# omarezz46/BayesDLL

Measured on AMD Instinct MI355X. Metric: SG-HMC leapfrog steps/sec & HBM GB/s on ViT-L/32 params, 1/2/4/8 MI355X, higher is better.
Workload: dtype f32

## Files before the change

### bayesdll_amd/csrc/bdl_api.hip

```cpp
#include <algorithm>
#include "bdl_chain_common.hpp"
#include "bdl_claim_ring.hpp"
#include "bdl_measure.h"

#include <mutex>
#include <vector>

namespace bdl {
namespace {

thread_local std::string g_last_error;

int g_blocks_per_cu = 2;
int g_unroll = 1;
int g_grid_stride = 1;

int device_cu_count() {
  static int cached[64] = {0};
  int dev = 0;
  if (hipGetDevice(&dev) != hipSuccess || dev < 0 || dev >= 64) return 256;
  if (cached[dev] == 0) {
    int cus = 0;
    if (hipDeviceGetAttribute(&cus, hipDeviceAttributeMultiprocessorCount, dev) != hipSuccess ||
        cus <= 0)
// ... 479 lines not shown
  if (!s) return fail(BDL_ERR_NULL, "bdl_sgmcmc_step: null args");
  if (s->n < 0) return fail(BDL_ERR_ARG, "bdl_sgmcmc_step: n < 0");
  if (s->method < BDL_CSGHMC || s->method > BDL_SGLD_GRAD)
    return fail(BDL_ERR_ARG, "bdl_sgmcmc_step: unknown method");
  if (s->noise_mode < BDL_NOISE_NONE || s->noise_mode > BDL_NOISE_PHILOX)
    return fail(BDL_ERR_ARG, "bdl_sgmcmc_step: unknown noise mode");
  if (s->collect < BDL_COLLECT_NONE || s->collect > BDL_COLLECT_MEAN)
    return fail(BDL_ERR_ARG, "bdl_sgmcmc_step: unknown collect mode");
  if (s->n == 0) return BDL_OK;
  const bool grad_only = s->method == BDL_SGHMC_GRAD || s->method == BDL_SGLD_GRAD;
  const bool needs_mom = s->method == BDL_CSGHMC || s->method == BDL_SGHMC ||
                         s->method == BDL_SGHMC_GRAD ||
                         (s->method == BDL_SGLD && (s->flags & BDL_FLAG_MOMENTUM));
  const bool needs_prior = s->method != BDL_CSGHMC;
  if (!s->theta) return fail(BDL_ERR_NULL, "bdl_sgmcmc_step: theta is required");
  if (const int rc = check_runs_and_grad(s, "bdl_sgmcmc_step")) return rc;
  if (needs_mom && !s->mom) return fail(BDL_ERR_NULL, "bdl_sgmcmc_step: mom is required");
  if (needs_prior && !s->prior_mean)
    return fail(BDL_ERR_NULL, "bdl_sgmcmc_step: prior_mean is required for sghmc/sgld");
  if (s->noise_mode == BDL_NOISE_BUFFER && !s->noise)
    return fail(BDL_ERR_NULL, "bdl_sgmcmc_step: noise buffer is required");
  if (s->collect != BDL_COLLECT_NONE && !s->mom1)
    return fail(BDL_ERR_NULL, "bdl_sgmcmc_step: mom1 is required to collect");
  if (grad_only && s->collect != BDL_COLLECT_NONE)
    return fail(BDL_ERR_ARG, "bdl_sgmcmc_step: grad-only methods cannot collect");
  const void* ptrs[] = {s->theta, s->mom, s->prior_mean, s->noise, s->mom1, s->mom2};
  for (const void* p : ptrs)
    if (misaligned(p, 15)) return fail(BDL_ERR_ALIGN, "bdl_sgmcmc_step: vector not 16-B aligned");

  const int unroll = g_unroll;
  StepKernel k = bare ? (s->method == BDL_CSGHMC ? pick_step_csghmc_bare(s->collect, unroll)
                                                 : nullptr)
                      : pick_step(s->method, s->noise_mode, s->collect, unroll);
  if (!k) return fail(BDL_ERR_ARG, "bdl_sgmcmc_step: unsupported method/noise/collect combination");

  const int64_t ngroups = (s->n + 3) / 4;
  const int64_t per_iter = (int64_t)kBlock * unroll;
  const int64_t cap = (int64_t)device_cu_count() * g_blocks_per_cu;
  int64_t iters = (ngroups + per_iter - 1) / per_iter;
  int64_t grid = capped_grid(iters, cap);
  int64_t iters_per_block = (iters + grid - 1) / grid;
  grid = (iters + iters_per_block - 1) / iters_per_block;

  KArgs a;
  a.theta = s->theta;
  a.grad = s->grad;
  a.mom = s->mom;
  a.prior_mean = s->prior_mean;
  a.noise = s->noise;
  a.mom1 = s->mom1;
  a.mom2 = s->mom2;
  a.runs = s->runs;
  a.gbase = s->grad_base;
  a.nruns = s->nruns;
  a.flags = s->flags;
  a.n = s->n;
  const int order = drift ? drift->order : g_grid_stride;
  a.groups_per_block = order ? 0 : iters_per_block * per_iter;
  a.lr0 = s->lr[0];
  a.lr1 = s->lr[1];
  a.ns0 = s->noise_scale[0];
  a.ns1 = s->noise_scale[1];
  a.one_minus_alpha = s->one_minus_alpha;
  a.prior_sig = s->prior_sig;
  a.sigma2 = s->sigma2;
  a.n_data = s->n_data;
  a.mu = s->mu;
  a.ca = s->collect_a;
  a.cb = s->collect_b;
  a.seed = s->seed;
  a.chain = s->chain;
  a.step = s->step;
  a.clip = clip;
  a.nonfinite = s->nonfinite;
  a.goff = s->philox_offset;
  a.cgroups = (uint32_t)s->chain_groups;
  a.inv_s2 = recip_or(s->inv_sigma2, s->sigma2);
  a.inv_nd = recip_or(s->inv_n_data, s->n_data);
  a.inv_ca = recip_or(s->inv_collect_a, s->collect_a);
  a.inv_cb = recip_or(s->inv_collect_b, s->collect_b);

  int slot = -1;
  uint32_t* pair = nullptr;
  if (order == 2 && s->method == BDL_CSGHMC &&
      run_lds_bytes(s) + 16 <= (size_t)kMaxRuns * sizeof(bdl_run))
    pair = claim_pair(stream, &slot);
  g_last_order = pair ? 2 : (order ? 1 : 0);
  g_last_slot = slot;
  const int32_t citers = (int32_t)(BDL_CLAIM_GROUPS / per_iter);
  if (pair) grid = capped_grid((iters + citers - 1) / citers, cap);
  if (drift) {
    if (order == 2 && !pair)
      return fail(BDL_ERR_ARG, "bdl_sweep_drift: no counter pair for the dynamic order here");
    if (drift->record_bytes < grid * (int64_t)(BDL_DRIFT_WORDS * sizeof(uint64_t)))
      return fail(BDL_ERR_ARG, "bdl_sweep_drift: records too small for the launch's workgroups");
    *drift->grid = (int32_t)grid;
    hipLaunchKernelGGL(pick_drift(unroll, pair != nullptr), dim3((unsigned)grid), dim3(kBlock),
                       run_lds_bytes(s), stream, a, pair, citers, drift->records);
    return launched("bdl_sweep_drift");
  }
  if (pair) {
    hipLaunchKernelGGL(pick_step_csghmc_dyn(s->noise_mode, s->collect, unroll, bare),
                       dim3((unsigned)grid), dim3(kBlock), run_lds_bytes(s), stream, a, pair, citers);
    return launched("bdl_sgmcmc_step");
  }

  if (g_redirect_exec) {
    hipGraphNodeType nt = hipGraphNodeTypeEmpty;
    hipKernelNodeParams cur{};
    if (hipGraphNodeGetType(g_redirect_node, &nt) != hipSuccess || nt != hipGraphNodeTypeKernel ||
        hipGraphKernelNodeGetParams(g_redirect_node, &cur) != hipSuccess ||
        cur.func != (void*)k) {
      (void)hipGetLastError();
      return fail(BDL_ERR_ARG, "bdl_sgmcmc_step: the redirect node is not this step's kernel");
    }
    void* kp[] = {&a};
    hipKernelNodeParams p{};
    p.func = (void*)k;
    p.gridDim = dim3((unsigned)grid);
    p.blockDim = dim3(kBlock);
    p.sharedMemBytes = (unsigned)run_lds_bytes(s);
    p.kernelParams = kp;
    const hipError_t err = hipGraphExecKernelNodeSetParams(g_redirect_exec, g_redirect_node, &p);
    if (err != hipSuccess) {
      (void)hipGetLastError();
      g_last_error = std::string("bdl_sgmcmc_step: graph node update failed: ") +
                     hipGetErrorString(err);
      return BDL_ERR_LAUNCH;
    }
    return BDL_OK;
  }
  hipLaunchKernelGGL(k, dim3((unsigned)grid), dim3(kBlock), run_lds_bytes(s), stream, a);
  if (const int rc = launched("bdl_sgmcmc_step")) return rc;
  hipStreamCaptureStatus cs = hipStreamCaptureStatusNone;
  if (stream && hipStreamIsCapturing(stream, &cs) == hipSuccess &&
      cs == hipStreamCaptureStatusActive) {
    std::lock_guard<std::mutex> lk(g_captured_mu);
    if (std::find(g_captured_funcs.begin(), g_captured_funcs.end(), (const void*)k) ==
        g_captured_funcs.end())
      g_captured_funcs.push_back((const void*)k);
  }
  (void)hipGetLastError();
  return BDL_OK;
}


constexpr int kMixMaxR = 8, kMixMaxW = 6;
struct MixArgs {
  const float* r[kMixMaxR];
  float* w[kMixMaxW];
  int64_t n;
};

template <int NR, int U>
__device__ __forceinline__ void mix_load(const MixArgs& a, int64_t gb, f4v (&x)[U][NR]) {
#pragma unroll
  for (int u = 0; u < U; ++u) {
    const int64_t e = (gb + (int64_t)u * kBlock + threadIdx.x) * 4;
#pragma unroll
    for (int r = 0; r < NR; ++r) x[u][r] = vload(a.r[r] + e);
  }
}

template <int NR, int NW, int U, bool PACED>
__device__ __forceinline__ void mix_store(const MixArgs& a, int64_t gb, f4v (&x)[U][NR]) {
#pragma unroll
  for (int u = 0; u < U; ++u) {
    const int64_t gi = gb + (int64_t)u * kBlock + threadIdx.x;
    const int64_t e = gi * 4;
    f4v acc = x[u][0];
#pragma unroll
    for (int r = 1; r < NR; ++r) acc = acc + x[u][r] * 0.0f;
    if constexpr (PACED) acc = acc + philox_normal4((uint64_t)gi, 0x5eedull, 0, 1) * 0.0f;
#pragma unroll
    for (int w = 0; w < NW; ++w) vstore(a.w[w] + e, acc);
  }
}

template <int NR, int NW, int U, int S>
__global__ __launch_bounds__(kBlock) void bdl_mix_kernel(const MixArgs a) {
  constexpr int64_t kIter = (int64_t)kBlock * U;
  const int64_t ngroups = (a.n + 3) >> 2, nfull = a.n >> 2;
  const int64_t stride = (int64_t)gridDim.x * kIter;
  int64_t gb = (int64_t)blockIdx.x * kIter;
  if constexpr (S == BDL_MIX_PIPELINED) {
    f4v x[U][NR], y[U][NR];
// ... 525 lines not shown
```

### bayesdll_amd/csrc/bdl_kernels.hpp

```cpp
#pragma once
#include <hip/hip_runtime.h>

#include <stdint.h>
#include <stdio.h>
#include <string.h>

#include <algorithm>
#include <string>

#include "bdl_sgmcmc.h"
#include "bdl_order.h"

namespace bdl {

constexpr int kBlock = 256;

__device__ __forceinline__ uint4 philox4x32_10(uint4 c, uint32_t k0, uint32_t k1) {
#ifdef BDL_PHILOX_KEYS_PER_CALL
  asm volatile("" : "+s"(k0), "+s"(k1));
#endif
#if defined(BDL_PHILOX_ROUND_KEYS_PER_CALL) && !defined(BDL_PHILOX_KEYS_PER_CALL)
  asm volatile("" : "+s"(k0), "+s"(k1));
#endif
#pragma unroll
// ... 555 lines not shown
  f4v th[UNROLL], g[UNROLL], v[UNROLL], t0[UNROLL], ep[UNROLL], m1[UNROLL], m2[UNROLL];
  uint32_t at[UNROLL];
  float* gq[UNROLL];
  const f4v z = {0.f, 0.f, 0.f, 0.f};
  int rr = r0;
#pragma unroll
  for (int u = 0; u < UNROLL; ++u) {
    const int64_t e = (gb + (int64_t)u * kBlock + threadIdx.x) * 4;
    while (run_end(rr) <= e) ++rr;
    at[u] = run_attr(rr);
    gq[u] = run_grad(a, rr);
    v[u] = t0[u] = ep[u] = m1[u] = m2[u] = z;
    th[u] = vload(a.theta + e);
    g[u] = vload(gq[u] + e);
    if (T::kMom || (METHOD == BDL_SGLD && c.sgd_mom_read)) v[u] = vload(a.mom + e);
    if (T::kReadPrior) t0[u] = vload(a.prior_mean + e);
    if (NOISE == BDL_NOISE_BUFFER) ep[u] = vload(a.noise + e);
    if (T::kReadMoments) {
      m1[u] = vload(a.mom1 + e);
      if (c.has_m2) m2[u] = vload(a.mom2 + e);
    }
  }
#pragma unroll
  for (int u = 0; u < UNROLL; ++u) {
    const int64_t gi = gb + (int64_t)u * kBlock + threadIdx.x;
    const int64_t e = gi * 4;
    if constexpr (NOISE == BDL_NOISE_PHILOX) ep[u] = step_noise4(a, gi);
#pragma unroll
    for (int j = 0; j < 4; ++j) {
      float xt = th[u][j], xg = g[u][j], xv = v[u][j], x1 = m1[u][j], x2 = m2[u][j];
      update_elem<METHOD, NOISE, COLLECT, RECIP>(a, c, at[u], xt, xg, xv, t0[u][j], ep[u][j], x1,
                                                 x2);
      th[u][j] = xt;
      g[u][j] = xg;
      v[u][j] = xv;
      m1[u][j] = x1;
      m2[u][j] = x2;
    }
    if constexpr (T::kWriteTheta) {
      bad |= nonfinite4(th[u]);
      vstore(a.theta + e, th[u]);
    }
    if constexpr (T::kWriteGrad) {
      bad |= nonfinite4(g[u]);
      vstore(gq[u] + e, g[u]);
    }
    if (T::kMom || (METHOD == BDL_SGLD && c.sgd_mom)) vstore(a.mom + e, v[u]);
    if constexpr (T::kCollect) {
      vstore(a.mom1 + e, m1[u]);
      if (c.has_m2) vstore(a.mom2 + e, m2[u]);
    }
  }
}

constexpr int kVarGradReady = 1, kVarClip = 2, kVarRuntime = -1;

template <int COLLECT, int UNROLL>
constexpr bool csg_collect_per_run() {
  return UNROLL == 1 &&
         (COLLECT == BDL_COLLECT_WELFORD_INIT || COLLECT == BDL_COLLECT_MEAN_INIT);
}

template <int METHOD, int COLLECT, int VAR, class A>
__device__ __forceinline__ StepConst make_step_const(const A& a) {
  StepConst c;
  c.sgd_mom = (METHOD == BDL_SGLD) && (a.flags & BDL_FLAG_MOMENTUM);
  c.sgd_mom_read = c.sgd_mom && !(a.flags & BDL_FLAG_FIRST_STEP);
  c.has_m2 = (COLLECT != BDL_COLLECT_NONE) && (a.mom2 != nullptr);
  if constexpr (VAR == kVarRuntime) {
    c.grad_ready = (METHOD == BDL_SGLD || METHOD == BDL_SGHMC) && (a.flags & BDL_FLAG_GRAD_READY);
    c.clip = (METHOD == BDL_SGLD) && a.clip != nullptr;
  } else {
    c.grad_ready = (VAR & kVarGradReady) != 0;
    c.clip = (VAR & kVarClip) != 0;
  }
  c.clip_coef = c.clip ? a.clip[1] : 1.0f;
  c.inv_s2 = a.inv_s2;
  c.inv_nd = a.inv_nd;
  c.inv_ca = a.inv_ca;
  c.inv_cb = a.inv_cb;
  return c;
}

template <int METHOD, int NOISE, int COLLECT, bool RECIP, int UNROLL, int VAR>
__device__ __forceinline__ void step_body(const KArgs& a) {
  const StepConst c = make_step_const<METHOD, COLLECT, VAR>(a);

  const int64_t ngroups = (a.n + 3) >> 2;
  const int64_t nfull = a.n >> 2;
  constexpr int64_t kIter = (int64_t)kBlock * UNROLL;
  int64_t g0, g1, gstep;
  if (a.groups_per_block > 0) {
    g0 = (int64_t)blockIdx.x * a.groups_per_block;
    g1 = min(g0 + a.groups_per_block, ngroups);
    gstep = kIter;
  } else {
    g0 = (int64_t)blockIdx.x * kIter;
    g1 = ngroups;
    gstep = (int64_t)gridDim.x * kIter;
  }

  stage_runs(a);
  if (g0 >= g1) return;

  int r = find_run_lds(a.nruns, g0 * 4);
  uint32_t bad = 0;
  if constexpr (fresh_step_args<METHOD, NOISE, COLLECT, UNROLL>()) {
  for (int64_t gb = g0; gb < g1; gb += gstep) {
    ckargs& fa = fresh_kargs();
    const StepConst fc = make_step_const<METHOD, COLLECT, VAR>(fa);
    while (r < a.nruns - 1 && run_end(r) <= gb * 4) ++r;
    const int64_t gend = min(gb + kIter, g1);
    const uint32_t attr = run_attr(r);
    const bool full = gend == gb + kIter && gend <= nfull;
    if (full && run_end(r) >= gend * 4 && !(attr & kNoFastPath))
      chunk_fast_dispatch<METHOD, NOISE, COLLECT, RECIP, UNROLL>(fa, fc, gb, attr, run_grad(fa, r),
                                                                  bad);
    else if (full && multi_run_ok(a.nruns, r, gend * 4))
      chunk_multi<METHOD, NOISE, COLLECT, RECIP, UNROLL>(fa, fc, gb, r, bad);
    else
      chunk_slow<METHOD, NOISE, COLLECT, RECIP, UNROLL>(fa, fc, gb, gend, r, bad);
  }
  } else if constexpr (!is_csghmc_sweep<METHOD>() ||
                       (COLLECT != BDL_COLLECT_NONE && !csg_collect_per_run<COLLECT, UNROLL>())) {
  for (int64_t gb = g0; gb < g1; gb += gstep) {
    while (r < a.nruns - 1 && run_end(r) <= gb * 4) ++r;
    const int64_t gend = min(gb + kIter, g1);
    const uint32_t attr = run_attr(r);
    const bool full = gend == gb + kIter && gend <= nfull;
    if (full && run_end(r) >= gend * 4 && !(attr & kNoFastPath))
      chunk_fast_dispatch<METHOD, NOISE, COLLECT, RECIP, UNROLL>(a, c, gb, attr, run_grad(a, r),
                                                                  bad);
    else if (full && multi_run_ok(a.nruns, r, gend * 4))
      chunk_multi<METHOD, NOISE, COLLECT, RECIP, UNROLL>(a, c, gb, r, bad);
    else
      chunk_slow<METHOD, NOISE, COLLECT, RECIP, UNROLL>(a, c, gb, gend, r, bad);
  }
  } else {
  for (int64_t gb = g0; gb < g1;) {
    while (r < a.nruns - 1 && run_end(r) <= gb * 4) ++r;
    const uint32_t attr = run_attr(r);
    const int64_t lim = min(min(run_end(r) >> 2, nfull), g1);
    if (!(attr & kNoFastPath) && gb + kIter <= lim) {
      const bool head = (attr & BDL_ATTR_HEAD) != 0;
      gb = fast_run<METHOD, NOISE, COLLECT, RECIP, UNROLL, false, false>(
          a, c, gb, lim, gstep, head ? a.lr1 : a.lr0, head ? a.ns1 : a.ns0, run_grad(a, r), bad);
      continue;
    }
    const int64_t gend = min(gb + kIter, g1);
    if (gend == gb + kIter && gend <= nfull && multi_run_ok(a.nruns, r, gend * 4))
      chunk_multi<METHOD, NOISE, COLLECT, RECIP, UNROLL>(a, c, gb, r, bad);
    else
      chunk_slow<METHOD, NOISE, COLLECT, RECIP, UNROLL>(a, c, gb, gend, r, bad);
    gb += gstep;
  }
  }
  report_nonfinite(a, bad);
}

template <int METHOD, int NOISE, int COLLECT, bool RECIP, int UNROLL>
__device__ __forceinline__ void step_variant(const KArgs& a) {
  if constexpr (COLLECT != BDL_COLLECT_NONE || !(METHOD == BDL_SGLD || METHOD == BDL_SGHMC)) {
    step_body<METHOD, NOISE, COLLECT, RECIP, UNROLL, kVarRuntime>(a);
  } else {
    if (a.flags & BDL_FLAG_GRAD_READY)
      step_body<METHOD, NOISE, COLLECT, RECIP, UNROLL, kVarGradReady>(a);
    else if (METHOD == BDL_SGLD && a.clip != nullptr)
      step_body<METHOD, NOISE, COLLECT, RECIP, UNROLL, kVarClip>(a);
    else
      step_body<METHOD, NOISE, COLLECT, RECIP, UNROLL, 0>(a);
  }
}

template <int METHOD, int NOISE, int COLLECT, int UNROLL>
__global__ __launch_bounds__(kBlock) void bdl_step_kernel(const KArgs a) {
  if (a.flags & BDL_FLAG_RECIP_DIV)
    step_variant<METHOD, NOISE, COLLECT, true, UNROLL>(a);
  else
    step_variant<METHOD, NOISE, COLLECT, false, UNROLL>(a);
}

struct NoProbe {
  __device__ __forceinline__ void begin() {}
  __device__ __forceinline__ void tick(int64_t) {}
  __device__ __forceinline__ void end() {}
};

struct DriftProbe {
  uint64_t* __restrict__ rec;
  uint32_t it;
  __device__ __forceinline__ void begin() {
    if (threadIdx.x == 0) rec[0] = wall_clock64();
  }
  __device__ __forceinline__ void tick(int64_t iter) {
    if (it % BDL_DRIFT_EVERY == 0) {
      const uint32_t s = it / BDL_DRIFT_EVERY;
      if (s < BDL_DRIFT_SAMPLES && threadIdx.x == 0) {
        rec[4 + 2 * s] = wall_clock64();
        rec[5 + 2 * s] = (uint64_t)iter;
      }
    }
    ++it;
  }
  __device__ __forceinline__ void end() {
    __threadfence();
    __syncthreads();
    if (threadIdx.x == 0) {
      rec[1] = wall_clock64();
      rec[2] = min((it + BDL_DRIFT_EVERY - 1) / BDL_DRIFT_EVERY, (uint32_t)BDL_DRIFT_SAMPLES);
      rec[3] = it;
    }
  }
};

template <int METHOD, int NOISE, int COLLECT, bool RECIP, int UNROLL, bool DYN, class PROBE>
__device__ __forceinline__ void csg_sweep(const KArgs& a, uint32_t* __restrict__ claim,
                                          int32_t citers, PROBE probe) {
  static_assert(is_csghmc_sweep<METHOD>(), "the dynamic order exists for the cSGHMC sweeps");
  __shared__ uint32_t s_claim[2];
  const StepConst c = make_step_const<METHOD, COLLECT, kVarRuntime>(a);
  const int64_t ngroups = (a.n + 3) >> 2;
  const int64_t nfull = a.n >> 2;
  constexpr int64_t kIter = (int64_t)kBlock * UNROLL;
  const int64_t cgroups = (int64_t)citers * kIter;
  int64_t g0, g1, gstep;
  if constexpr (DYN) {
    g0 = (int64_t)blockIdx.x * cgroups;
    g1 = min(g0 + cgroups, ngroups);
    gstep = kIter;
  } else if (a.groups_per_block > 0) {
    g0 = (int64_t)blockIdx.x * a.groups_per_block;
    g1 = min(g0 + a.groups_per_block, ngroups);
    gstep = kIter;
  } else {
    g0 = (int64_t)blockIdx.x * kIter;
    g1 = ngroups;
    gstep = (int64_t)gridDim.x * kIter;
  }
  stage_runs(a);
  probe.begin();
  uint32_t bad = 0, nxt = 0;
  int r = -1, par = 0;
  while (g0 < g1) {
    if constexpr (DYN) {
      if (threadIdx.x == 0) nxt = gridDim.x + atomicAdd(claim, 1u);
    }
    if (r < 0) r = find_run_lds(a.nruns, g0 * 4);
    if constexpr (COLLECT != BDL_COLLECT_NONE && !csg_collect_per_run<COLLECT, UNROLL>()) {
      for (int64_t gb = g0; gb < g1; gb += gstep) {
        while (r < a.nruns - 1 && run_end(r) <= gb * 4) ++r;
        const int64_t gend = min(gb + kIter, g1);
        const uint32_t attr = run_attr(r);
        const bool full = gend == gb + kIter && gend <= nfull;
        if (full && run_end(r) >= gend * 4 && !(attr & kNoFastPath))
          chunk_fast_dispatch<METHOD, NOISE, COLLECT, RECIP, UNROLL>(a, c, gb, attr,
                                                                      run_grad(a, r), bad);
        else if (full && multi_run_ok(a.nruns, r, gend * 4))
          chunk_multi<METHOD, NOISE, COLLECT, RECIP, UNROLL>(a, c, gb, r, bad);
        else
          chunk_slow<METHOD, NOISE, COLLECT, RECIP, UNROLL>(a, c, gb, gend, r, bad);
        probe.tick(gb / kIter);
      }
    } else {
      for (int64_t gb = g0; gb < g1;) {
        while (r < a.nruns - 1 && run_end(r) <= gb * 4) ++r;
        const uint32_t attr = run_attr(r);
        const int64_t lim = min(min(run_end(r) >> 2, nfull), g1);
        if (!(attr & kNoFastPath) && gb + kIter <= lim) {
          const bool head = (attr & BDL_ATTR_HEAD) != 0;
          const float eta = head ? a.lr1 : a.lr0, ns = head ? a.ns1 : a.ns0;
          float* gp = run_grad(a, r);
          do {
            chunk_fast<METHOD, NOISE, COLLECT, RECIP, UNROLL, false, false>(a, c, gb, eta, ns, gp,
                                                                            bad);
            probe.tick(gb / kIter);
            gb += gstep;
          } while (gb + kIter <= lim);
          continue;
        }
        const int64_t gend = min(gb + kIter, g1);
        if (gend == gb + kIter && gend <= nfull && multi_run_ok(a.nruns, r, gend * 4))
          chunk_multi<METHOD, NOISE, COLLECT, RECIP, UNROLL>(a, c, gb, r, bad);
        else
          chunk_slow<METHOD, NOISE, COLLECT, RECIP, UNROLL>(a, c, gb, gend, r, bad);
        probe.tick(gb / kIter);
        gb += gstep;
      }
    }
    if constexpr (!DYN) {
      break;
    } else {
      if (threadIdx.x == 0) s_claim[par] = nxt;
      __syncthreads();
      const uint32_t blk = s_claim[par];
      par ^= 1;
      g0 = (int64_t)blk * cgroups;
      g1 = min(g0 + cgroups, ngroups);
    }
  }
  report_nonfinite(a, bad);
  probe.end();
  if constexpr (DYN) {
    if (threadIdx.x == 0 && atomicAdd(claim + 1, 1u) == gridDim.x - 1) {
      __hip_atomic_store(claim, 0u, __ATOMIC_RELAXED, __HIP_MEMORY_SCOPE_AGENT);
      __hip_atomic_store(claim + 1, 0u, __ATOMIC_RELAXED, __HIP_MEMORY_SCOPE_AGENT);
    }
  }
}

template <int METHOD, int NOISE, int COLLECT, int UNROLL>
__global__ __launch_bounds__(kBlock) void bdl_step_dyn_kernel(const KArgs a, uint32_t* claim,
                                                              int32_t citers) {
  if (a.flags & BDL_FLAG_RECIP_DIV)
    csg_sweep<METHOD, NOISE, COLLECT, true, UNROLL, true, NoProbe>(a, claim, citers, NoProbe{});
  else
    csg_sweep<METHOD, NOISE, COLLECT, false, UNROLL, true, NoProbe>(a, claim, citers, NoProbe{});
}

template <int UNROLL, bool DYN>
__global__ __launch_bounds__(kBlock) void bdl_drift_kernel(const KArgs a, uint32_t* claim,
                                                           int32_t citers, uint64_t* rec) {
  DriftProbe p{rec + (size_t)blockIdx.x * BDL_DRIFT_WORDS, 0};
  if (a.flags & BDL_FLAG_RECIP_DIV)
    csg_sweep<BDL_CSGHMC, BDL_NOISE_NONE, BDL_COLLECT_NONE, true, UNROLL, DYN, DriftProbe>(
        a, claim, citers, p);
  else
    csg_sweep<BDL_CSGHMC, BDL_NOISE_NONE, BDL_COLLECT_NONE, false, UNROLL, DYN, DriftProbe>(
        a, claim, citers, p);
}

struct AdamConst {
  bool sgd_mom, sgd_mom_read, has_m2, grad_is_mom;
  float inv_s2, inv_nd, inv_temp, inv_bc1, inv_bc2, inv_ca, inv_cb;
};

template <int NOISE, bool RECIP, bool PRIOR, bool GRADONLY, class A>
__device__ __forceinline__ void adam_core(const A& a, const AdamConst& c, float eta, float& th,
                                          float& g, float& vm, float& m, float& v, float& buf,
                                          float th0, float eps) {
  const float gs = sdiv<RECIP>(g, a.temp, c.inv_temp);
  float gU = gs;
  if constexpr (PRIOR) {
    const float d = th - th0;
    const float e = sdiv<RECIP>(d, a.sigma2, c.inv_s2);
    gU = gs + sdiv<RECIP>(e, a.n_data, c.inv_nd);
  }
  m = m * a.b1 + gU * a.omb1;
  v = v * a.b2 + (gU * gU) * a.omb2;
  const float mh = sdiv<RECIP>(m, a.bc1, c.inv_bc1);
  const float vh = sdiv<RECIP>(v, a.bc2, c.inv_bc2);
  const float den = sqrtf(vh) + a.aeps;
  const float pg = mh / den;
  const float pt = 1.0f / den;
  float nz = 0.0f;
  if constexpr (NOISE != BDL_NOISE_NONE) {
    const float q = sdiv<RECIP>(pt * a.two_alpha, a.n_data, c.inv_nd);
    nz = (sqrtf(q) * a.nd) * eps;
  }
  vm = (vm * a.one_minus_alpha + pg * eta) + nz;
  const float gp = c.grad_is_mom ? vm : g + vm;
  if constexpr (GRADONLY) {
    g = gp;
  } else {
    float stepv = gp;
    if (c.sgd_mom) {
      buf = (a.flags & BDL_FLAG_FIRST_STEP) ? gp : (a.mu * buf + gp);
      stepv = buf;
    }
    th = fmaf(-eta, stepv, th);
  }
}

template <int NOISE, int COLLECT, bool RECIP, bool GRADONLY, bool PRIOR, int U>
__device__ __forceinline__ void adam_fast(const KArgs& a, const AdamConst& c, int64_t gb,
                                          float eta, float* gp, uint32_t& bad) {
  constexpr bool kReadMoments = (COLLECT == BDL_COLLECT_MEAN);
  const f4v z = {0.f, 0.f, 0.f, 0.f};
  f4v th[U], g[U], vm[U], m[U], v[U], buf[U], t0[U], ep[U], m1[U], m2[U];
#pragma unroll
  for (int u = 0; u < U; ++u) {
    const int64_t gi = gb + (int64_t)u * kBlock + threadIdx.x;
    const int64_t e = gi * 4;
    buf[u] = t0[u] = ep[u] = m1[u] = m2[u] = z;
    th[u] = vload(a.theta + e);
    g[u] = vload(gp + e);
    vm[u] = vload(a.mom + e);
    m[u] = vload(a.adam_m + e);
    v[u] = vload(a.adam_v + e);
    if (!GRADONLY && c.sgd_mom_read) buf[u] = vload(a.sgd_buf + e);
    if constexpr (PRIOR) t0[u] = vload(a.prior_mean + e);
    if constexpr (NOISE == BDL_NOISE_BUFFER) ep[u] = vload(a.noise + e);
    if constexpr (kReadMoments) {
// ... 395 lines not shown
    const int64_t gend = min(gb + kIter, ngroups);
    const uint32_t attr = run_attr(r);
    if (gend == gb + kIter && gend <= nfull && run_end(r) >= gend * 4 && !(attr & kNoFastPath)) {
      const float eta = (attr & BDL_ATTR_HEAD) ? a.lr1 : a.lr0;
      if (attr & BDL_ATTR_PRIOR)
        adam_fast<NOISE, COLLECT, RECIP, GRADONLY, true, U>(a, c, gb, eta, run_grad(a, r), bad);
      else
        adam_fast<NOISE, COLLECT, RECIP, GRADONLY, false, U>(a, c, gb, eta, run_grad(a, r), bad);
    } else {
      if (gend == gb + kIter && gend <= nfull && multi_run_ok(a.nruns, r, gend * 4))
        adam_multi<NOISE, COLLECT, RECIP, GRADONLY, U>(a, c, gb, r, bad);
      else
        adam_slow<NOISE, COLLECT, RECIP, GRADONLY, U>(a, c, gb, gend, r, bad);
    }
  }
  report_nonfinite(a, bad);
}

template <int NOISE, int COLLECT, bool GRADONLY, int U>
__global__ __launch_bounds__(kBlock) void bdl_adam_kernel(const KArgs a) {
  if (a.flags & BDL_FLAG_RECIP_DIV)
    adam_body<NOISE, COLLECT, true, GRADONLY, U>(a);
  else
    adam_body<NOISE, COLLECT, false, GRADONLY, U>(a);
}

using StepKernel = void (*)(const KArgs);

template <int METHOD, int NOISE, int COLLECT>
StepKernel pick_unroll(int unroll) {
  constexpr bool kAllDepths =
      is_csghmc_sweep<METHOD>() ||
      ((METHOD == BDL_SGLD || METHOD == BDL_SGHMC) && NOISE != BDL_NOISE_NONE);
  if constexpr (!kAllDepths) {
    (void)unroll;
    return bdl_step_kernel<METHOD, NOISE, COLLECT, 2>;
  } else {
    switch (unroll) {
      case 1:
        return bdl_step_kernel<METHOD, NOISE, COLLECT, 1>;
      case 4:
        return bdl_step_kernel<METHOD, NOISE, COLLECT, 4>;
      default:
        return bdl_step_kernel<METHOD, NOISE, COLLECT, 2>;
    }
  }
}

template <int METHOD, int NOISE>
StepKernel pick_collect(int collect, int unroll) {
  switch (collect) {
    case BDL_COLLECT_NONE:
      return pick_unroll<METHOD, NOISE, BDL_COLLECT_NONE>(unroll);
    case BDL_COLLECT_WELFORD_INIT:
      return pick_unroll<METHOD, NOISE, BDL_COLLECT_WELFORD_INIT>(unroll);
    case BDL_COLLECT_WELFORD:
      return pick_unroll<METHOD, NOISE, BDL_COLLECT_WELFORD>(unroll);
    case BDL_COLLECT_MEAN_INIT:
      return pick_unroll<METHOD, NOISE, BDL_COLLECT_MEAN_INIT>(unroll);
    case BDL_COLLECT_MEAN:
      return pick_unroll<METHOD, NOISE, BDL_COLLECT_MEAN>(unroll);
  }
  return nullptr;
}

template <int METHOD>
StepKernel pick_noise(int noise, int collect, int unroll) {
  switch (noise) {
    case BDL_NOISE_NONE:
      return pick_collect<METHOD, BDL_NOISE_NONE>(collect, unroll);
    case BDL_NOISE_BUFFER:
      return pick_collect<METHOD, BDL_NOISE_BUFFER>(collect, unroll);
    case BDL_NOISE_PHILOX:
      return pick_collect<METHOD, BDL_NOISE_PHILOX>(collect, unroll);
  }
  return nullptr;
}

StepKernel pick_step_csghmc(int noise, int collect, int unroll);
StepKernel pick_step_csghmc_bare(int collect, int unroll);
using DynKernel = void (*)(const KArgs, uint32_t*, int32_t);
using DriftKernel = void (*)(const KArgs, uint32_t*, int32_t, uint64_t*);
DynKernel pick_step_csghmc_dyn(int noise, int collect, int unroll, bool bare);
DriftKernel pick_drift(int unroll, bool dyn);
StepKernel pick_step_sghmc(int method, int noise, int collect, int unroll);
StepKernel pick_step_sgld(int method, int noise, int collect, int unroll);
StepKernel pick_adam(int noise, int collect, bool grad_only, int unroll);

}
```

### bayesdll_amd/kernels.py

```python
from __future__ import annotations

import ctypes as C
import os

import numpy as np
import torch

from . import _lib as L
from . import ess as E

DIV_MODE = os.environ.get("BDL_DIV_MODE", "recip")


def _div_flag(div_mode=None):
    return L.FLAG_RECIP_DIV if (div_mode or DIV_MODE) == "recip" else 0


def _inv(s):
    s = float(s)
    return 1.0 / s if s != 0.0 else 0.0


def _step_args(state, method, *, lrs, noise_scale, noise_mode, one_minus_alpha=1.0,
               prior_sig=0.0, sigma2=1.0, n_data=1.0, mu=0.0, first_step=False,
# ... 1722 lines not shown
        nonfinite_per_chain = nf is not None and nf.numel() == int(state.K) and int(state.K) > 1
    a.nonfinite_per_chain = 1 if nonfinite_per_chain else 0
    a.mom = None if state.mom is None else state.mom.data_ptr()
    a.prior_mean = None if state.prior is None else state.prior.data_ptr()
    nz = noise if noise is not None else getattr(state, "noise", None)
    a.noise = None if nz is None else nz.data_ptr()
    a.mom1 = None if mom1 is None else mom1.data_ptr()
    a.mom2 = None if mom2 is None else mom2.data_ptr()
    a.runs = state.chain_runs.data_ptr()
    a.nruns = int(state.chain_nruns)
    a.scalars = scalars.data_ptr()
    a.n1, a.chain_groups, a.chains = int(state.n1), int(state.chain_groups), int(state.K)
    a.method, a.noise_mode, a.collect = int(method), int(noise_mode), int(collect)
    a.flags = ((L.FLAG_FIRST_STEP if first_step else 0) | (L.FLAG_MOMENTUM if momentum else 0)
               | _div_flag(div_mode))
    a.blocks_per_chain, a.unroll = int(blocks_per_chain), int(unroll)
    a.collect_a, a.collect_b = float(collect_a), float(collect_b)
    a.inv_collect_a, a.inv_collect_b = _inv(collect_a), _inv(collect_b)
    a.seed = int(seed) & 0xFFFFFFFFFFFFFFFF
    a.chain = int(chain) & 0xFFFFFFFFFFFFFFFF
    a.step = int(step) & 0xFFFFFFFFFFFFFFFF
    return a


def chain_step(state, method, *, scalars, **kw):
    K_ = int(state.K)
    if (scalars.dtype != torch.float32 or not scalars.is_cuda or not scalars.is_contiguous()
            or scalars.numel() != K_ * 12 or scalars.device != state.theta.device):
        raise ValueError("chain_step: scalars must be a contiguous float32 [K, 12] tensor on the "
                         "state's device")
    if not kw.get("blocks_per_chain"):
        kw["blocks_per_chain"] = chain_step_blocks_per_chain(state.n1, K_, state.theta.device,
                                                             kw.get("unroll") or 1)
    a = chain_step_args(state, method, scalars=scalars, **kw)
    dev = state.theta.device
    t = getattr(state, "timer", None)
    e0 = t.begin() if t is not None else None
    L.check(L.lib().bdl_chain_step(a, L.current_stream_handle(dev)), "bdl_chain_step")
    if e0 is not None:
        t.end(e0, alg_bytes_per_elem(a) * int(a.n1) * K_)


def philox_normal(n, seed, chain, step, device="cuda"):
    out = torch.empty(n, dtype=torch.float32, device=device)
    L.check(L.lib().bdl_philox_normal(out.data_ptr(), int(n), int(seed), int(chain), int(step),
                                      L.current_stream_handle(out.device)), "bdl_philox_normal")
    return out


_ACTIVE = [None]
LIBRARY_DEFAULT = (2, 1, 1)


def set_launch_config(blocks_per_cu=0, unroll=0, grid_stride=0):
    _ACTIVE[0] = (int(blocks_per_cu), int(unroll), int(grid_stride))
    return L.lib().bdl_set_launch_config(int(blocks_per_cu), int(unroll), int(grid_stride))


def restore_launch_config(packed):
    return set_launch_config((packed >> 8) & 0xFFFF, packed & 0xFF, (packed >> 24) & 0xFF)


def _use_geometry(state, kind="step", sub=False):
    cfg = getattr(state, {"collect": "collect_cfg", "init": "init_cfg"}.get(kind, "launch_cfg"),
                  None)
    if cfg is None:
        cfg = getattr(state, "launch_cfg", None)
    if sub:
        act = cfg or _ACTIVE[0]
        if act is not None and act[2] == L.ORDER_DYNAMIC:
            cfg = (act[0], act[1], L.ORDER_GRID_STRIDE)
    if cfg is not None and cfg != _ACTIVE[0]:
        set_launch_config(*cfg)


AUTOTUNE_CANDIDATES = ((2, 1, 1), (1, 4, 1), (3, 1, 1), (2, 4, 1), (1, 2, 1), (2, 2, 1))
AUTOTUNE_BY_METHOD = {
    "csghmc": (AUTOTUNE_CANDIDATES + ((3, 4, 1), (1, 1, 1))
               + tuple((b, u, L.ORDER_DYNAMIC)
                       for b, u, _ in AUTOTUNE_CANDIDATES + ((3, 4, 1), (1, 1, 1)))),
    "sgld": AUTOTUNE_CANDIDATES + ((3, 4, 1), (4, 4, 1), (1, 1, 1)),
    "adam": AUTOTUNE_CANDIDATES + ((1, 1, 1), (4, 4, 1)),
}
_TUNED = {}
_TUNED_COLLECT = {}
COLLECT_EXTRA = ((1, 1, 1),)


ADAM_EXTRA = ("adam_m", "adam_v", "sgd_buf")


def _scratch_launcher(n, dev, method):
    return _scratch_launchers(n, dev, method)[0]


def _scratch_launchers(n, dev, method):
    from .flat import FlatState, moment_pair
    st = FlatState.from_segments([("w", (int(n),))], None, device=dev,
                                 need_prior=method != "csghmc",
                                 extra=ADAM_EXTRA if method == "adam" else ())
    st.theta.zero_()
    if method == "csghmc":
        kw = dict(lrs=(1e-4, 1e-4), noise_scale=(0.0, 0.0), noise_mode=L.NOISE_NONE,
                  one_minus_alpha=0.9, prior_sig=1.0)

        def launch():
            sgmcmc_step(st, L.CSGHMC, **kw)
    elif method == "sgld":
        st.prior.zero_()
        kw = dict(lrs=(1e-4, 1e-4), noise_scale=(1e-3, 1e-3), noise_mode=L.NOISE_PHILOX,
                  sigma2=1.0, n_data=1e6, mu=0.5, momentum=True)

        def launch():
            sgmcmc_step(st, L.SGLD, **kw)
    elif method == "adam":
        st.prior.zero_()
        m, v, buf = (st.extra[k] for k in ADAM_EXTRA)
        kw = dict(adam_m=m, adam_v=v, sgd_buf=buf, beta1=0.9, beta2=0.999, eps=1e-8, t=3,
                  momentum_decay=0.1, nd=0.01, lrs=(1e-4, 1e-4), noise_mode=L.NOISE_PHILOX,
                  sigma2=1.0, n_data=1e6, mu=0.5, momentum=True)

        def launch():
            adam_step(st, L.ADAM_SGHMC, **kw)
    else:
        raise ValueError(f"unknown method {method!r}")
    moms = []

    def launch_collect():
        if not moms:
            moms.extend(moment_pair(int(n), dev) if method == "csghmc" else
                        (torch.zeros_like(st.theta), torch.zeros_like(st.theta)))
            moms[0].copy_(st.theta)
            moms[1].zero_()
        if method == "csghmc":
            sgmcmc_step(st, L.CSGHMC, lrs=(1e-4, 1e-4), noise_scale=(1e-7, 1e-7),
                        noise_mode=L.NOISE_PHILOX, one_minus_alpha=0.9, prior_sig=1.0,
                        collect=L.COLLECT_WELFORD, mom1=moms[0], mom2=moms[1], collect_a=3.0)
        elif method == "sgld":
            sgmcmc_step(st, L.SGLD, collect=L.COLLECT_MEAN, mom1=moms[0], mom2=moms[1],
                        collect_a=2.0, collect_b=3.0, **kw)
        else:
            adam_step(st, L.ADAM_SGHMC, collect=L.COLLECT_MEAN, mom1=moms[0], mom2=moms[1],
                      collect_a=2.0, collect_b=3.0, **kw)
    return launch, launch_collect


def _device(device):
    return torch.device(device) if device is not None else torch.device(
        "cuda", torch.cuda.current_device())


def autotune(n, device=None, reps=6, candidates=None, method="csghmc", collect=False):
    import numpy as np
    dev = _device(device)
    if candidates is None:
        candidates = AUTOTUNE_BY_METHOD.get(method, AUTOTUNE_CANDIDATES)
    launch, launch_collect = _scratch_launchers(n, dev, method)

    def pick(fn, cands):
        times = measure(fn, cands, reps)
        top = sorted(times, key=times.get)[:3]
        again = measure(fn, top, 2 * reps)
        for cfg in top:
            times[cfg] = 0.5 * (times[cfg] + again[cfg])
        return min(top, key=times.get), times

    def measure(fn, cfgs, k):
        out = {}
        for cfg in cfgs:
            set_launch_config(*cfg)
            for _ in range(2):
                fn()
            ev = [(torch.cuda.Event(enable_timing=True), torch.cuda.Event(enable_timing=True))
                  for _ in range(k)]
            for e0, e1 in ev:
                e0.record()
                fn()
                e1.record()
            torch.cuda.synchronize(dev)
            out[cfg] = float(np.median([a.elapsed_time(b) for a, b in ev]))
        return out

    best, times = pick(launch, candidates)
    res = (best, times)
    if collect:
        cbest, ctimes = pick(launch_collect, tuple(candidates) + tuple(
            c for c in COLLECT_EXTRA if c not in candidates))
        res = (best, times, cbest, ctimes)
    set_launch_config(*best)
    del launch, launch_collect
    torch.cuda.empty_cache()
    return res


TUNE_ON_STATE_MIN = 1 << 16
TUNE_SNAPSHOT_FRACTION = 0.25


def request_state_tuning(state, method):
    if os.environ.get("BDL_AUTOTUNE", "1") == "0" or int(state.n) < TUNE_ON_STATE_MIN:
        return
    state._tune_pending = {"step", "collect", "init"}
    state._tune_method = method
    state.tuned = {}


def _tune_kind(state, fn, kind, written):
    state._tune_pending.discard(kind)
    cands = tuple(AUTOTUNE_BY_METHOD.get(state._tune_method, AUTOTUNE_CANDIDATES))
    if kind != "step":
        cands += tuple(c for c in COLLECT_EXTRA if c not in cands)
    nf = getattr(state, "nonfinite", None)
    written = list(written) + ([nf] if nf is not None else [])
    need = sum(w.numel() * w.element_size() for w in written)
    free, _ = torch.cuda.mem_get_info(state.device)
    if need > TUNE_SNAPSHOT_FRACTION * free:
        state.tuned[kind] = {"skipped": f"snapshot {need >> 20} MiB > "
                                        f"{TUNE_SNAPSHOT_FRACTION:g} x free {free >> 20} MiB"}
        return
    best, times = tune_on_state(fn, written, cands, state.device)
    setattr(state, {"collect": "collect_cfg", "init": "init_cfg"}.get(kind, "launch_cfg"), best)
    state.tuned[kind] = {"best": best,
                         "ms": {f"{c[0]}wg/cu x{c[1]}" + (" dynamic" if c[2] == L.ORDER_DYNAMIC
                                                          else ""): round(t, 4)
                                for c, t in times.items()}}


def tune_on_state(launch, written, candidates, device, reps=4):
    import numpy as np
    saved = [w.clone() for w in written]
    prev = _ACTIVE[0]
    ts = torch.cuda.current_stream(device)

    def measure(cfgs, k):
        out = {}
        for cfg in cfgs:
            set_launch_config(*cfg)
            launch()
            ev = [(torch.cuda.Event(enable_timing=True), torch.cuda.Event(enable_timing=True))
                  for _ in range(k)]
            for e0, e1 in ev:
                e0.record(ts)
                launch()
                e1.record(ts)
            torch.cuda.synchronize(device)
            out[cfg] = float(np.median([x.elapsed_time(y) for x, y in ev]))
            for w, s in zip(written, saved):
                w.copy_(s)
        return out

    try:
        times = measure(candidates, reps)
        top = sorted(times, key=times.get)[:3]
        again = measure(top, 2 * reps)
        for cfg in top:
            times[cfg] = 0.5 * (times[cfg] + again[cfg])
        best = min(top, key=times.get)
    finally:
        for w, s in zip(written, saved):
            w.copy_(s)
        del saved
        if prev is not None:
            set_launch_config(*prev)
    return best, times


def prewarm(n, device=None, method="csghmc", seconds=2.5):
    import time
    dev = _device(device)
    launch = _scratch_launcher(n, dev, method)
    t_end, k = time.perf_counter() + float(seconds), 0
    while time.perf_counter() < t_end:
        for _ in range(20):
            launch()
        k += 20
        torch.cuda.synchronize(dev)
    del launch
    torch.cuda.empty_cache()
    return k


def autotune_once(n, device, method):
    if os.environ.get("BDL_AUTOTUNE", "1") == "0":
        return None
    key = (int(n), str(device), method)
    if key not in _TUNED:
        best, _, cbest, _ = autotune(n, device, method=method, collect=True)
        _TUNED[key], _TUNED_COLLECT[key] = best, cbest
    else:
        set_launch_config(*_TUNED[key])
    return _TUNED[key]

# ... 4 lines not shown
```

Before: 1025.

## Extend dynamic work-claiming sweep order to SGLD and SGHMC step kernels

Adds a dynamic-order sweep kernel for SGLD and SGHMC in which workgroups claim chunks through an atomic counter pair, as the cSGHMC path already does. The host launcher routes to it when the dynamic order is selected and the step is not bare, drift-probed, clipped or grad-ready. The autotuner offers dynamic-order candidates only for SGLD states of at least 2^27 elements. The aim is to balance load across workgroups on large parameter vectors, at the cost of atomics, per-chunk syncs and more kernel instantiations.

```diff
diff --git a/bayesdll_amd/csrc/bdl_api.hip b/bayesdll_amd/csrc/bdl_api.hip
--- a/bayesdll_amd/csrc/bdl_api.hip
+++ b/bayesdll_amd/csrc/bdl_api.hip
@@ -585,8 +585,11 @@
 
   int slot = -1;
   uint32_t* pair = nullptr;
-  if (order == 2 && s->method == BDL_CSGHMC &&
-      run_lds_bytes(s) + 16 <= (size_t)kMaxRuns * sizeof(bdl_run))
+  const bool dyn_method =
+      s->method == BDL_CSGHMC ||
+      ((s->method == BDL_SGLD || s->method == BDL_SGHMC) && !bare && !drift && !clip &&
+       !(s->flags & BDL_FLAG_GRAD_READY));
+  if (order == 2 && dyn_method && run_lds_bytes(s) + 16 <= (size_t)kMaxRuns * sizeof(bdl_run))
     pair = claim_pair(stream, &slot);
   g_last_order = pair ? 2 : (order ? 1 : 0);
   g_last_slot = slot;
@@ -603,8 +606,12 @@
     return launched("bdl_sweep_drift");
   }
   if (pair) {
-    hipLaunchKernelGGL(pick_step_csghmc_dyn(s->noise_mode, s->collect, unroll, bare),
-                       dim3((unsigned)grid), dim3(kBlock), run_lds_bytes(s), stream, a, pair, citers);
+    const DynKernel dk =
+        s->method == BDL_SGLD    ? pick_step_sgld_dyn(s->noise_mode, s->collect, unroll)
+        : s->method == BDL_SGHMC ? pick_step_sghmc_dyn(s->noise_mode, s->collect, unroll)
+                                 : pick_step_csghmc_dyn(s->noise_mode, s->collect, unroll, bare);
+    hipLaunchKernelGGL(dk, dim3((unsigned)grid), dim3(kBlock), run_lds_bytes(s), stream, a, pair,
+                       citers);
     return launched("bdl_sgmcmc_step");
   }
 
diff --git a/bayesdll_amd/csrc/bdl_kernels.hpp b/bayesdll_amd/csrc/bdl_kernels.hpp
--- a/bayesdll_amd/csrc/bdl_kernels.hpp
+++ b/bayesdll_amd/csrc/bdl_kernels.hpp
@@ -661,6 +661,22 @@
   return c;
 }
 
+template <int METHOD, int NOISE, int COLLECT, bool RECIP, int UNROLL, class A>
+__device__ __forceinline__ void block_iter(const A& a, const StepConst& c, int nruns, int64_t gb,
+                                           int64_t g1, int64_t nfull, int& r, uint32_t& bad) {
+  constexpr int64_t kIter = (int64_t)kBlock * UNROLL;
+  while (r < nruns - 1 && run_end(r) <= gb * 4) ++r;
+  const int64_t gend = min(gb + kIter, g1);
+  const uint32_t attr = run_attr(r);
+  const bool full = gend == gb + kIter && gend <= nfull;
+  if (full && run_end(r) >= gend * 4 && !(attr & kNoFastPath))
+    chunk_fast_dispatch<METHOD, NOISE, COLLECT, RECIP, UNROLL>(a, c, gb, attr, run_grad(a, r), bad);
+  else if (full && multi_run_ok(nruns, r, gend * 4))
+    chunk_multi<METHOD, NOISE, COLLECT, RECIP, UNROLL>(a, c, gb, r, bad);
+  else
+    chunk_slow<METHOD, NOISE, COLLECT, RECIP, UNROLL>(a, c, gb, gend, r, bad);
+}
+
 template <int METHOD, int NOISE, int COLLECT, bool RECIP, int UNROLL, int VAR>
 __device__ __forceinline__ void step_body(const KArgs& a) {
   const StepConst c = make_step_const<METHOD, COLLECT, VAR>(a);
@@ -791,6 +807,25 @@
     }
   }
 };
+
+__device__ __forceinline__ uint32_t claim_issue(uint32_t* __restrict__ claim) {
+  return gridDim.x + atomicAdd(claim, 1u);
+}
+
+__device__ __forceinline__ uint32_t claim_take(uint32_t* s_claim, int& par, uint32_t nxt) {
+  if (threadIdx.x == 0) s_claim[par] = nxt;
+  __syncthreads();
+  const uint32_t blk = s_claim[par];
+  par ^= 1;
+  return blk;
+}
+
+__device__ __forceinline__ void claim_done(uint32_t* __restrict__ claim) {
+  if (threadIdx.x == 0 && atomicAdd(claim + 1, 1u) == gridDim.x - 1) {
+    __hip_atomic_store(claim, 0u, __ATOMIC_RELAXED, __HIP_MEMORY_SCOPE_AGENT);
+    __hip_atomic_store(claim + 1, 0u, __ATOMIC_RELAXED, __HIP_MEMORY_SCOPE_AGENT);
+  }
+}
 
 template <int METHOD, int NOISE, int COLLECT, bool RECIP, int UNROLL, bool DYN, class PROBE>
 __device__ __forceinline__ void csg_sweep(const KArgs& a, uint32_t* __restrict__ claim,
@@ -887,6 +922,50 @@
   }
 }
 
+template <int METHOD, int NOISE, int COLLECT, bool RECIP, int UNROLL>
+__device__ __forceinline__ void step_sweep_dyn(const KArgs& a, uint32_t* __restrict__ claim,
+                                               int32_t citers) {
+  static_assert(METHOD == BDL_SGLD || METHOD == BDL_SGHMC, "the step methods other than cSGHMC");
+  __shared__ uint32_t s_claim[2];
+  const StepConst c = make_step_const<METHOD, COLLECT, 0>(a);
+  const int64_t ngroups = (a.n + 3) >> 2;
+  const int64_t nfull = a.n >> 2;
+  constexpr int64_t kIter = (int64_t)kBlock * UNROLL;
+  const int64_t cgroups = (int64_t)citers * kIter;
+  int64_t g0 = (int64_t)blockIdx.x * cgroups;
+  int64_t g1 = min(g0 + cgroups, ngroups);
+  stage_runs(a);
+  uint32_t bad = 0, nxt = 0;
+  int r = -1, par = 0;
+  while (g0 < g1) {
+    if (threadIdx.x == 0) nxt = claim_issue(claim);
+    if (r < 0) r = find_run_lds(a.nruns, g0 * 4);
+    for (int64_t gb = g0; gb < g1; gb += kIter) {
+      if constexpr (fresh_step_args<METHOD, NOISE, COLLECT, UNROLL>()) {
+        ckargs& fa = fresh_kargs();
+        const StepConst fc = make_step_const<METHOD, COLLECT, 0>(fa);
+        block_iter<METHOD, NOISE, COLLECT, RECIP, UNROLL>(fa, fc, a.nruns, gb, g1, nfull, r, bad);
+      } else {
+        block_iter<METHOD, NOISE, COLLECT, RECIP, UNROLL>(a, c, a.nruns, gb, g1, nfull, r, bad);
+      }
+    }
+    const uint32_t blk = claim_take(s_claim, par, nxt);
+    g0 = (int64_t)blk * cgroups;
+    g1 = min(g0 + cgroups, ngroups);
+  }
+  report_nonfinite(a, bad);
+  claim_done(claim);
+}
+
+template <int METHOD, int NOISE, int COLLECT, int UNROLL>
+__global__ __launch_bounds__(kBlock) void bdl_step_sweep_dyn_kernel(const KArgs a, uint32_t* claim,
+                                                               int32_t citers) {
+  if (a.flags & BDL_FLAG_RECIP_DIV)
+    step_sweep_dyn<METHOD, NOISE, COLLECT, true, UNROLL>(a, claim, citers);
+  else
+    step_sweep_dyn<METHOD, NOISE, COLLECT, false, UNROLL>(a, claim, citers);
+}
+
 template <int METHOD, int NOISE, int COLLECT, int UNROLL>
 __global__ __launch_bounds__(kBlock) void bdl_step_dyn_kernel(const KArgs a, uint32_t* claim,
                                                               int32_t citers) {
@@ -1448,6 +1527,50 @@
 using DynKernel = void (*)(const KArgs, uint32_t*, int32_t);
 using DriftKernel = void (*)(const KArgs, uint32_t*, int32_t, uint64_t*);
 DynKernel pick_step_csghmc_dyn(int noise, int collect, int unroll, bool bare);
+DynKernel pick_step_sgld_dyn(int noise, int collect, int unroll);
+DynKernel pick_step_sghmc_dyn(int noise, int collect, int unroll);
+
+template <int METHOD, int NOISE, int COLLECT>
+DynKernel pick_dyn_unroll(int unroll) {
+  switch (unroll) {
+    case 1:
+      return bdl_step_sweep_dyn_kernel<METHOD, NOISE, COLLECT, 1>;
+    case 4:
+      return bdl_step_sweep_dyn_kernel<METHOD, NOISE, COLLECT, 4>;
+    default:
+      return bdl_step_sweep_dyn_kernel<METHOD, NOISE, COLLECT, 2>;
+  }
+}
+
+template <int METHOD, int NOISE>
+DynKernel pick_dyn_collect(int collect, int unroll) {
+  switch (collect) {
+    case BDL_COLLECT_NONE:
+      return pick_dyn_unroll<METHOD, NOISE, BDL_COLLECT_NONE>(unroll);
+    case BDL_COLLECT_WELFORD_INIT:
+      return pick_dyn_unroll<METHOD, NOISE, BDL_COLLECT_WELFORD_INIT>(unroll);
+    case BDL_COLLECT_WELFORD:
+      return pick_dyn_unroll<METHOD, NOISE, BDL_COLLECT_WELFORD>(unroll);
+    case BDL_COLLECT_MEAN_INIT:
+      return pick_dyn_unroll<METHOD, NOISE, BDL_COLLECT_MEAN_INIT>(unroll);
+    case BDL_COLLECT_MEAN:
+      return pick_dyn_unroll<METHOD, NOISE, BDL_COLLECT_MEAN>(unroll);
+  }
+  return nullptr;
+}
+
+template <int METHOD>
+DynKernel pick_dyn_noise(int noise, int collect, int unroll) {
+  switch (noise) {
+    case BDL_NOISE_NONE:
+      return pick_dyn_collect<METHOD, BDL_NOISE_NONE>(collect, unroll);
+    case BDL_NOISE_BUFFER:
+      return pick_dyn_collect<METHOD, BDL_NOISE_BUFFER>(collect, unroll);
+    case BDL_NOISE_PHILOX:
+      return pick_dyn_collect<METHOD, BDL_NOISE_PHILOX>(collect, unroll);
+  }
+  return nullptr;
+}
 DriftKernel pick_drift(int unroll, bool dyn);
 StepKernel pick_step_sghmc(int method, int noise, int collect, int unroll);
 StepKernel pick_step_sgld(int method, int noise, int collect, int unroll);
diff --git a/bayesdll_amd/csrc/bdl_step_sghmc_dyn.hip b/bayesdll_amd/csrc/bdl_step_sghmc_dyn.hip
--- /dev/null
+++ b/bayesdll_amd/csrc/bdl_step_sghmc_dyn.hip
@@ -0,0 +1,9 @@
+#include "bdl_kernels.hpp"
+
+namespace bdl {
+
+DynKernel pick_step_sghmc_dyn(int noise, int collect, int unroll) {
+  return pick_dyn_noise<BDL_SGHMC>(noise, collect, unroll);
+}
+
+}
diff --git a/bayesdll_amd/csrc/bdl_step_sgld_dyn.hip b/bayesdll_amd/csrc/bdl_step_sgld_dyn.hip
--- /dev/null
+++ b/bayesdll_amd/csrc/bdl_step_sgld_dyn.hip
@@ -0,0 +1,9 @@
+#include "bdl_kernels.hpp"
+
+namespace bdl {
+
+DynKernel pick_step_sgld_dyn(int noise, int collect, int unroll) {
+  return pick_dyn_noise<BDL_SGLD>(noise, collect, unroll);
+}
+
+}
diff --git a/bayesdll_amd/kernels.py b/bayesdll_amd/kernels.py
--- a/bayesdll_amd/kernels.py
+++ b/bayesdll_amd/kernels.py
@@ -1828,6 +1828,17 @@
     "sgld": AUTOTUNE_CANDIDATES + ((3, 4, 1), (4, 4, 1), (1, 1, 1)),
     "adam": AUTOTUNE_CANDIDATES + ((1, 1, 1), (4, 4, 1)),
 }
+DYNAMIC_ORDER_METHODS = ("sgld",)
+DYNAMIC_ORDER_MIN_N = 1 << 27
+
+
+def tune_candidates(method, n):
+    cands = tuple(AUTOTUNE_BY_METHOD.get(method, AUTOTUNE_CANDIDATES))
+    if method in DYNAMIC_ORDER_METHODS and int(n) >= DYNAMIC_ORDER_MIN_N:
+        cands += tuple((b, u, L.ORDER_DYNAMIC) for b, u, o in cands if o == L.ORDER_GRID_STRIDE)
+    return cands
+
+
 _TUNED = {}
 _TUNED_COLLECT = {}
 COLLECT_EXTRA = ((1, 1, 1),)
@@ -1953,7 +1964,7 @@
 
 def _tune_kind(state, fn, kind, written):
     state._tune_pending.discard(kind)
-    cands = tuple(AUTOTUNE_BY_METHOD.get(state._tune_method, AUTOTUNE_CANDIDATES))
+    cands = tune_candidates(state._tune_method, state.n)
     if kind != "step":
         cands += tuple(c for c in COLLECT_EXTRA if c not in cands)
     nf = getattr(state, "nonfinite", None)
```

Measured after the change: 1000. -2.4%, worse.
